# Adttil/crypto12381

Hardware: AMD Instinct MI355X
Metric: G1 scalar-muls/s per MI355X (batch 2^20 per GPU), bit-exact vs CPU (higher is better)
Workload: dtype int64 accumulate over 14x28-bit signed limbs

## Files before the change

crypto12381_amd/csrc/fp.hpp:

```cpp
#pragma once
#include <cstdint>
#include <type_traits>
#include <utility>

#if defined(__HIPCC__)
#include <hip/hip_runtime.h>
#define C12381_HD __host__ __device__ __forceinline__
#define C12381_HDN __host__ __device__ __noinline__ inline
#define C12381_CONST __device__ constexpr
#else
#define C12381_HD inline
#define C12381_HDN inline
#define C12381_CONST constexpr
#endif

#if defined(__HIP_DEVICE_COMPILE__)
#define C12381_LIMB(x) c12381::limb_opaque(x)
namespace c12381 { __device__ __forceinline__ int32_t limb_opaque(int32_t v) { asm("" : "+v"(v)); return v; } }
#else
#define C12381_LIMB(x) (x)
#endif

#include "consts.hpp"

// ... 176 lines not shown
    int64_t acc = 0;
#pragma unroll
    for (int k = 0; k < NL; ++k) {
#pragma unroll
        for (int i = 0; 2 * i < k; ++i) { acc += (int64_t)a2[i] * a.l[k - i]; }
        if ((k & 1) == 0) { acc += (int64_t)a.l[k / 2] * a.l[k / 2]; }
#pragma unroll
        for (int i = 0; i < k; ++i) { acc += (int64_t)m[i] * FP_P[k - i]; }
        m[k] = (int32_t)(((uint32_t)acc * FP_N0) & LMASK);
        acc += (int64_t)m[k] * FP_P[0];
        acc >>= LB;
    }
#pragma unroll
    for (int k = NL; k < 2 * NL - 1; ++k) {
#pragma unroll
        for (int i = k - NL + 1; 2 * i < k; ++i) { acc += (int64_t)a2[i] * a.l[k - i]; }
        if ((k & 1) == 0) { acc += (int64_t)a.l[k / 2] * a.l[k / 2]; }
#pragma unroll
        for (int i = k - NL + 1; i < NL; ++i) { acc += (int64_t)m[i] * FP_P[k - i]; }
        out[k - NL] = C12381_LIMB((int32_t)((uint32_t)acc & LMASK));
        acc >>= LB;
    }
    out[NL - 1] = (int32_t)acc;
#pragma unroll
    for (int i = 0; i < NL; ++i) r.l[i] = out[i];
    C12381_BOUNDS({ double vb = a.vb * a.vb * P_OVER_R + 1.0;
                    double top = vb * TOP_PER_P + 2.0;
                    set_bounds(r, top > 268435456.0 ? top : 268435456.0, vb, "fp_sqr"); })
}

C12381_HD void fp_sqr2(fp& r, const fp& a) {
    C12381_BOUNDS({ fp d;
                    for (int i = 0; i < NL; ++i) d.l[i] = 2 * a.l[i];
                    d.lb = 2 * a.lb; d.vb = 2 * a.vb;
                    check_mul_operands(a, d, "fp_sqr2"); })
    C12381_COUNT(27, 1);
    int32_t m[NL];
    int32_t out[NL];
    int32_t a2[NL];
#pragma unroll
    for (int i = 0; i < NL; ++i) a2[i] = 2 * a.l[i];
    int64_t acc = 0;
#pragma unroll
    for (int k = 0; k < NL; ++k) {
#pragma unroll
        for (int i = 0; 2 * i < k; ++i) { acc += (int64_t)a2[i] * a2[k - i]; }
        if ((k & 1) == 0) { acc += (int64_t)a2[k / 2] * a.l[k / 2]; }
#pragma unroll
        for (int i = 0; i < k; ++i) { acc += (int64_t)m[i] * FP_P[k - i]; }
        m[k] = (int32_t)(((uint32_t)acc * FP_N0) & LMASK);
        acc += (int64_t)m[k] * FP_P[0];
        acc >>= LB;
    }
#pragma unroll
    for (int k = NL; k < 2 * NL - 1; ++k) {
#pragma unroll
        for (int i = k - NL + 1; 2 * i < k; ++i) { acc += (int64_t)a2[i] * a2[k - i]; }
        if ((k & 1) == 0) { acc += (int64_t)a2[k / 2] * a.l[k / 2]; }
#pragma unroll
        for (int i = k - NL + 1; i < NL; ++i) { acc += (int64_t)m[i] * FP_P[k - i]; }
        out[k - NL] = C12381_LIMB((int32_t)((uint32_t)acc & LMASK));
        acc >>= LB;
    }
    out[NL - 1] = (int32_t)acc;
#pragma unroll
    for (int i = 0; i < NL; ++i) r.l[i] = out[i];
    C12381_BOUNDS({ double vb = 2 * a.vb * a.vb * P_OVER_R + 1.0;
                    double top = vb * TOP_PER_P + 2.0;
                    set_bounds(r, top > 268435456.0 ? top : 268435456.0, vb, "fp_sqr2"); })
}

C12381_HD void fp_col_acc(int64_t& acc, const fp& a, const fp& b, int k) {
    C12381_COUNT(1, 0);
#pragma unroll
    for (int i = 0; i < NL; ++i) {
        const int j = k - i;
        if (j >= 0 && j < NL) { acc += (int64_t)a.l[i] * b.l[j]; }
    }
}
C12381_HD void fp_col_sqr_acc(int64_t& acc, const fp& a, const fp& a2, const fp& ad, int k) {
    C12381_COUNT(1, 0);
#pragma unroll
    for (int i = 0; i < NL; ++i) {
        const int j = k - i;
        if (j > i && j < NL) { acc += (int64_t)a2.l[i] * a.l[j]; }
    }
    if ((k & 1) == 0 && k / 2 < NL) { acc += (int64_t)ad.l[k / 2] * a.l[k / 2]; }
}
C12381_HD void fp_raw_neg(fp& r, const fp& a) {
#pragma unroll
    for (int i = 0; i < NL; ++i) r.l[i] = -a.l[i];
    C12381_BOUNDS(r.lb = a.lb; r.vb = a.vb;)
}
C12381_HD void fp_raw_dbl(fp& r, const fp& a) {
#pragma unroll
    for (int i = 0; i < NL; ++i) r.l[i] = 2 * a.l[i];
    C12381_BOUNDS(r.lb = 2 * a.lb; r.vb = 2 * a.vb;)
}
C12381_HD void fp_raw_neg_dbl(fp& r, const fp& a) {
#pragma unroll
    for (int i = 0; i < NL; ++i) r.l[i] = -2 * a.l[i];
    C12381_BOUNDS(r.lb = 2 * a.lb; r.vb = 2 * a.vb;)
}
template <class ColFn>
C12381_HD void fp_reduce_cols(fp& r, ColFn col) {
    C12381_COUNT(0, 1);
    int32_t m[NL];
    int32_t out[NL];
    int64_t acc = 0;
#pragma unroll
    for (int k = 0; k < NL; ++k) {
        col(k, acc);
#pragma unroll
        for (int i = 0; i < k; ++i) { acc += (int64_t)m[i] * FP_P[k - i]; }
        m[k] = (int32_t)(((uint32_t)acc * FP_N0) & LMASK);
        acc += (int64_t)m[k] * FP_P[0];
        acc >>= LB;
    }
#pragma unroll
    for (int k = NL; k < 2 * NL - 1; ++k) {
        col(k, acc);
#pragma unroll
        for (int i = k - NL + 1; i < NL; ++i) { acc += (int64_t)m[i] * FP_P[k - i]; }
        out[k - NL] = C12381_LIMB((int32_t)((uint32_t)acc & LMASK));
        acc >>= LB;
    }
    out[NL - 1] = (int32_t)acc;
#pragma unroll
    for (int i = 0; i < NL; ++i) r.l[i] = out[i];
}
template <int... Ks, class Fn>
C12381_HD void fp_static_for(std::integer_sequence<int, Ks...>, Fn&& fn) { (fn(std::integral_constant<int, Ks>{}), ...); }
template <class ColFn>
C12381_HD void fp_reduce_cols_static(fp& r, ColFn col) {
    C12381_COUNT(0, 1);
    int32_t m[NL];
    int32_t out[NL];
    int64_t acc = 0;
    fp_static_for(std::make_integer_sequence<int, NL>{}, [&](auto kc) {
        constexpr int k = decltype(kc)::value;
        col(k, acc);
#pragma unroll
        for (int i = 0; i < k; ++i) { acc += (int64_t)m[i] * FP_P[k - i]; }
        m[k] = (int32_t)(((uint32_t)acc * FP_N0) & LMASK);
        acc += (int64_t)m[k] * FP_P[0];
        acc >>= LB;
    });
    fp_static_for(std::make_integer_sequence<int, NL - 1>{}, [&](auto kc) {
        constexpr int k = NL + decltype(kc)::value;
        col(k, acc);
#pragma unroll
        for (int i = k - NL + 1; i < NL; ++i) { acc += (int64_t)m[i] * FP_P[k - i]; }
        out[k - NL] = C12381_LIMB((int32_t)((uint32_t)acc & LMASK));
        acc >>= LB;
    });
    out[NL - 1] = (int32_t)acc;
#pragma unroll
    for (int i = 0; i < NL; ++i) r.l[i] = out[i];
}
C12381_HD void fp_inj(int64_t& acc, const fp& c, int i, int32_t k) { acc += (int64_t)c.l[i] * k; }
C12381_HD void fp_inj_p(int64_t& acc, int i, int32_t k) { acc += (int64_t)FP_P[i] * k; }
C12381_HD int32_t fp_quot_top(int32_t top) { return (int32_t)(((int64_t)top * 1321315992 + ((int64_t)1 << 46)) >> 47); }
#if defined(__HIP_DEVICE_COMPILE__)
C12381_HD int32_t fp_opaque_const(int32_t v) { asm("" : "+s"(v)); return v; }
#else
C12381_HD int32_t fp_opaque_const(int32_t v) { return v; }
#endif
template <class ColFn, class InjFn>
C12381_HD void fp_reduce_cols_inj(fp& r, ColFn col, InjFn inj) {
    C12381_COUNT(0, 1);
    int32_t m[NL];
    int32_t out[NL];
    int64_t acc = 0;
#pragma unroll
    for (int k = 0; k < NL; ++k) {
        col(k, acc);
#pragma unroll
        for (int i = 0; i < k; ++i) { acc += (int64_t)m[i] * FP_P[k - i]; }
        m[k] = (int32_t)(((uint32_t)acc * FP_N0) & LMASK);
        acc += (int64_t)m[k] * FP_P[0];
        acc >>= LB;
    }
#pragma unroll
    for (int k = NL; k < 2 * NL - 1; ++k) {
        col(k, acc);
        inj(k - NL, acc);
#pragma unroll
        for (int i = k - NL + 1; i < NL; ++i) { acc += (int64_t)m[i] * FP_P[k - i]; }
        out[k - NL] = C12381_LIMB((int32_t)((uint32_t)acc & LMASK));
        acc >>= LB;
    }
    inj(NL - 1, acc);
    out[NL - 1] = (int32_t)acc;
#pragma unroll
    for (int i = 0; i < NL; ++i) r.l[i] = out[i];
}
template <class InjFn>
C12381_HD void fp_mul_inj(fp& r, const fp& a, const fp& b, InjFn inj, double inj_vb, double inj_lb) {
    C12381_COUNT(27, 0);
    fp t;
    fp_reduce_cols_inj(t, [&](int k, int64_t& acc) {
#pragma unroll
        for (int i = 0; i < NL; ++i) { const int j = k - i; if (j >= 0 && j < NL) { acc += (int64_t)a.l[i] * b.l[j]; } }
    }, inj);
    (void)inj_vb; (void)inj_lb;
    C12381_BOUNDS({ check_actual(a, "fp_mul_inj"); check_actual(b, "fp_mul_inj"); set_inj_bounds(t, a.lb * b.lb, a.vb * b.vb, inj_vb, inj_lb, "fp_mul_inj"); })
    r = t;
}
template <class InjFn>
C12381_HD void fp_sqr_inj(fp& r, const fp& a, InjFn inj, double inj_vb, double inj_lb) {
    C12381_COUNT(27, 0);
    fp t, a2;
    fp_raw_dbl(a2, a);
    fp_reduce_cols_inj(t, [&](int k, int64_t& acc) {
#pragma unroll
        for (int i = 0; i < NL; ++i) { const int j = k - i; if (j > i && j < NL) { acc += (int64_t)a2.l[i] * a.l[j]; } }
        if ((k & 1) == 0 && k / 2 < NL) { acc += (int64_t)a.l[k / 2] * a.l[k / 2]; }
    }, inj);
    (void)inj_vb; (void)inj_lb;
    C12381_BOUNDS({ check_actual(a, "fp_sqr_inj"); set_inj_bounds(t, a.lb * a.lb, a.vb * a.vb, inj_vb, inj_lb, "fp_sqr_inj"); })
    r = t;
}
C12381_HD void fp_norm1_dbl(fp& r, const fp& a) {
    int32_t c[NL];
#pragma unroll
    for (int i = 0; i < NL - 1; ++i) c[i] = a.l[i] >> (LB - 1);
    const int32_t t13 = 2 * a.l[NL - 1] + c[NL - 2];
#pragma unroll
    for (int i = NL - 2; i >= 1; --i) r.l[i] = C12381_LIMB((int32_t)(((uint32_t)a.l[i] << 1) & LMASK)) + c[i - 1];
    r.l[0] = C12381_LIMB((int32_t)(((uint32_t)a.l[0] << 1) & LMASK));
    r.l[NL - 1] = t13;
    C12381_BOUNDS({ double top = 2 * a.vb * TOP_PER_P + 6.0 + std::floor(2 * a.lb / 268435456.0);
                    double lb = 268435456.0 + std::floor(2 * a.lb / 268435456.0) + 1.0;
                    set_bounds(r, lb > top ? lb : top, 2 * a.vb, "fp_norm1_dbl"); })
}

C12381_HD void fp_lincomb3p(fp& r, const fp& a, int32_t k0, const fp& b, int32_t k1, const fp& c, int32_t k2, int32_t kp, double vb) {
    int64_t t = 0;
    int32_t out[NL];
#pragma unroll
    for (int i = 0; i < NL - 1; ++i) {
        t += (int64_t)a.l[i] * k0; t += (int64_t)b.l[i] * k1; t += (int64_t)c.l[i] * k2; t += (int64_t)FP_P[i] * kp;
        out[i] = C12381_LIMB((int32_t)((uint32_t)t & LMASK));
        t >>= LB;
    }
    t += (int64_t)a.l[NL - 1] * k0; t += (int64_t)b.l[NL - 1] * k1; t += (int64_t)c.l[NL - 1] * k2; t += (int64_t)FP_P[NL - 1] * kp;
    out[NL - 1] = (int32_t)t;
#pragma unroll
    for (int i = 0; i < NL; ++i) r.l[i] = out[i];
    (void)vb;
    C12381_BOUNDS({ double top = vb * TOP_PER_P + 2.0;
                    set_bounds(r, top > 268435456.0 ? top : 268435456.0, vb, "fp_lincomb3p"); check_actual_vb(r, "fp_lincomb3p value"); })
}

template <bool SUB>
C12381_HD void fp_mul2(fp& r, const fp& a, const fp& b, const fp& c, const fp& d);

#ifdef C12381_CHECK_BOUNDS
inline void set_lazy_bounds(fp& r, double sum_lblb, double sum_vbvb, const char* where) {
    double col = 14.0 * sum_lblb + 14.0 * 72057594037927936.0 + 1099511627776.0;
    if (col >= 9223372036854775808.0) bounds_fail(where, sum_lblb, sum_vbvb);
    if (sum_vbvb > 1.0e6) bounds_fail("lazy form value bound", sum_vbvb, 0);
    double vb = sum_vbvb * P_OVER_R + 1.0;
    double top = vb * TOP_PER_P + 2.0;
    set_bounds(r, top > 268435456.0 ? top : 268435456.0, vb, where);
}
inline void set_inj_bounds(fp& r, double sum_lblb, double sum_vbvb, double inj_abs, double inj_lb, const char* where) {
    double col = 14.0 * sum_lblb + 14.0 * 72057594037927936.0 + 1099511627776.0 + inj_lb;
    if (col >= 9223372036854775808.0) bounds_fail(where, sum_lblb, inj_lb);
    if (sum_vbvb > 1.0e6) bounds_fail("injected form value bound", sum_vbvb, 0);
    double vb = sum_vbvb * P_OVER_R + 1.0 + inj_abs;
    double top = vb * TOP_PER_P + 2.0;
    set_bounds(r, top > 268435456.0 ? top : 268435456.0, vb, where);
    check_actual_vb(r, where);
}
inline double fp_actual_vb(const fp& a) {
    long double v = 0, w = 1;
    for (int i = 0; i < NL; ++i) { v += (long double)a.l[i] * w; w *= 268435456.0L; }
    long double pp = 0; w = 1;
    for (int i = 0; i < NL; ++i) { pp += (long double)FP_P[i] * w; w *= 268435456.0L; }
    return (double)fabsl(v / pp);
}
inline void check_actual_vb(const fp& a, const char* where) { const double v = fp_actual_vb(a); if (v > a.vb * 1.0000001 + 1e-9) bounds_fail(where, v, a.vb); }
#endif

template <bool SUB>
C12381_HD void fp_mul2(fp& r, const fp& a, const fp& b, const fp& c, const fp& d) {
    fp t, cs;
    if (SUB) fp_raw_neg(cs, c); else cs = c;
    fp_reduce_cols(t, [&](int k, int64_t& acc) { fp_col_acc(acc, a, b, k); fp_col_acc(acc, cs, d, k); });
    C12381_BOUNDS({ check_actual(a, "fp_mul2"); check_actual(b, "fp_mul2"); check_actual(c, "fp_mul2"); check_actual(d, "fp_mul2");
                    set_lazy_bounds(t, a.lb * b.lb + c.lb * d.lb, a.vb * b.vb + c.vb * d.vb, "fp_mul2"); })
    r = t;
}
C12381_HD void fp_mul_msqr2(fp& r, const fp& a, const fp& b, const fp& c) {
    fp t, c2, c4;
    fp_raw_neg_dbl(c2, c);
    fp_raw_dbl(c4, c2);
    fp_reduce_cols(t, [&](int k, int64_t& acc) { fp_col_acc(acc, a, b, k); fp_col_sqr_acc(acc, c, c4, c2, k); });
    C12381_BOUNDS({ check_actual(a, "fp_mul_msqr2"); check_actual(b, "fp_mul_msqr2"); check_actual(c, "fp_mul_msqr2");
                    set_lazy_bounds(t, a.lb * b.lb + 2 * c.lb * c.lb, a.vb * b.vb + 2 * c.vb * c.vb, "fp_mul_msqr2"); })
    r = t;
}

C12381_HD void fp_from_mont_canonical(fp& r, const fp& a) {
    fp one;
    fp_zero(one);
    one.l[0] = 1;
    C12381_BOUNDS(one.lb = 1; one.vb = 1e-100;)
    fp t;
    fp_mul(t, a, one);
    bool eqp = true;
#pragma unroll
    for (int i = 0; i < NL; ++i) eqp = eqp && (t.l[i] == FP_P[i]);
#pragma unroll
    for (int i = 0; i < NL; ++i) r.l[i] = eqp ? 0 : t.l[i];
    C12381_BOUNDS(r.lb = 268435456.0; r.vb = 1.0;)
}
C12381_HD bool fp_is_zero(const fp& a) {
    fp t;
    fp_from_mont_canonical(t, a);
    int32_t o = 0;
#pragma unroll
    for (int i = 0; i < NL; ++i) o |= t.l[i];
    return o == 0;
}
C12381_HD bool fp_equal(const fp& a, const fp& b) {
    fp d;
    fp_sub(d, a, b);
    return fp_is_zero(d);
}

C12381_HD void fp_from_words_be(fp& r, const uint32_t (&w)[12]) {
    fp t;
#pragma unroll
    for (int i = 0; i < NL; ++i) {
        const int bit = i * LB;
        const int wi = bit / 32, sh = bit % 32;
        uint64_t lo = w[11 - wi];
        if (wi + 1 < 12) lo |= (uint64_t)w[11 - (wi + 1)] << 32;
        t.l[i] = C12381_LIMB((int32_t)((uint32_t)(lo >> sh) & LMASK));
    }
    C12381_BOUNDS(t.lb = 268435456.0; t.vb = 10.0;)
    fp r2;
    fp_set_const(r2, FP_R2);
    fp_mul(r, t, r2);
}
C12381_HD void fp_to_words_be(uint32_t (&w)[12], const fp& a) {
    fp t;
    fp_from_mont_canonical(t, a);
#pragma unroll
    for (int j = 0; j < 12; ++j) {
        const int bit = j * 32;
        const int li = bit / LB, sh = bit % LB;
        uint64_t v = (uint64_t)(uint32_t)t.l[li] >> sh;
        if (li + 1 < NL) v |= (uint64_t)(uint32_t)t.l[li + 1] << (LB - sh);
        if (li + 2 < NL && 2 * LB - sh < 32) v |= (uint64_t)(uint32_t)t.l[li + 2] << (2 * LB - sh);
        w[11 - j] = (uint32_t)v;
    }
}
C12381_HD int fp_sign(const fp& a) {
    fp t;
    fp_from_mont_canonical(t, a);
    return t.l[0] & 1;
}

C12381_HDN void fp_pow_fixed(fp& r, const fp& a, const uint32_t (&e)[12]) {
    fp tab[16];
    fp_one(tab[0]);
    {
        fp n;
        fp_norm1(n, a);
        tab[1] = n;
    }
#pragma unroll 1
    for (int i = 2; i < 16; ++i) fp_mul(tab[i], tab[i - 1], tab[1]);
    fp acc;
    fp_one(acc);
#pragma unroll 1
    for (int wi = 95; wi >= 0; --wi) {
        fp_sqr(acc, acc); fp_sqr(acc, acc); fp_sqr(acc, acc); fp_sqr(acc, acc);
        const uint32_t d = (e[wi / 8] >> (4 * (wi % 8))) & 15u;
        fp_mul(acc, acc, tab[d]);
    }
    r = acc;
}
C12381_HD void fp_inv_fermat(fp& r, const fp& a) { fp_pow_fixed(r, a, EXP_P_MINUS_2); }

constexpr int SG_N = 13;
struct sg30 { int32_t v[SG_N]; };
C12381_HD int32_t sg_divsteps_30(int32_t zeta, uint32_t f0, uint32_t g0, int32_t (&t)[4]) {
    uint32_t u = 1, v = 0, q = 0, r = 1, f = f0, g = g0;
#pragma unroll 1
    for (int i = 0; i < 30; ++i) {
        uint32_t c1 = (uint32_t)(zeta >> 31);
        const uint32_t c2 = (uint32_t)0 - (g & 1u);
        const uint32_t x = (f ^ c1) - c1, y = (u ^ c1) - c1, z = (v ^ c1) - c1;
        g += x & c2; q += y & c2; r += z & c2;
        c1 &= c2;
        zeta = (int32_t)((uint32_t)zeta ^ c1) - 1;
        f += g & c1; u += q & c1; v += r & c1;
        g >>= 1; u <<= 1; v <<= 1;
    }
    t[0] = (int32_t)u; t[1] = (int32_t)v; t[2] = (int32_t)q; t[3] = (int32_t)r;
    return zeta;
}
C12381_HD void sg_update_de(sg30& d, sg30& e, const int32_t (&t)[4]) {
    constexpr int32_t M30 = (int32_t)0x3fffffff;
    const int32_t u = t[0], v = t[1], q = t[2], r = t[3];
    const int32_t sd = d.v[SG_N - 1] >> 31, se = e.v[SG_N - 1] >> 31;
    int32_t md = (u & sd) + (v & se), me = (q & sd) + (r & se);
    int32_t di = d.v[0], ei = e.v[0];
    int64_t cd = (int64_t)u * di + (int64_t)v * ei;
    int64_t ce = (int64_t)q * di + (int64_t)r * ei;
    md -= (int32_t)((SG_PINV30 * (uint32_t)cd + (uint32_t)md) & (uint32_t)M30);
    me -= (int32_t)((SG_PINV30 * (uint32_t)ce + (uint32_t)me) & (uint32_t)M30);
    cd += (int64_t)SG_P30[0] * md;
    ce += (int64_t)SG_P30[0] * me;
    cd >>= 30; ce >>= 30;
#pragma unroll
    for (int i = 1; i < SG_N; ++i) {
        di = d.v[i]; ei = e.v[i];
        cd += (int64_t)u * di + (int64_t)v * ei;
        ce += (int64_t)q * di + (int64_t)r * ei;
        cd += (int64_t)SG_P30[i] * md;
        ce += (int64_t)SG_P30[i] * me;
        d.v[i - 1] = (int32_t)cd & M30; cd >>= 30;
        e.v[i - 1] = (int32_t)ce & M30; ce >>= 30;
    }
    d.v[SG_N - 1] = (int32_t)cd; e.v[SG_N - 1] = (int32_t)ce;
}
C12381_HD void sg_update_fg(sg30& f, sg30& g, const int32_t (&t)[4]) {
    constexpr int32_t M30 = (int32_t)0x3fffffff;
    const int32_t u = t[0], v = t[1], q = t[2], r = t[3];
    int32_t fi = f.v[0], gi = g.v[0];
    int64_t cf = (int64_t)u * fi + (int64_t)v * gi;
    int64_t cg = (int64_t)q * fi + (int64_t)r * gi;
    cf >>= 30; cg >>= 30;
#pragma unroll
    for (int i = 1; i < SG_N; ++i) {
        fi = f.v[i]; gi = g.v[i];
        cf += (int64_t)u * fi + (int64_t)v * gi;
        cg += (int64_t)q * fi + (int64_t)r * gi;
        f.v[i - 1] = (int32_t)cf & M30; cf >>= 30;
        g.v[i - 1] = (int32_t)cg & M30; cg >>= 30;
    }
    f.v[SG_N - 1] = (int32_t)cf; g.v[SG_N - 1] = (int32_t)cg;
}
C12381_HD void sg_normalize(sg30& r, int32_t sign) {
    constexpr int32_t M30 = (int32_t)0x3fffffff;
    int32_t w[SG_N];
#pragma unroll
    for (int i = 0; i < SG_N; ++i) w[i] = r.v[i];
    int32_t cond_add = w[SG_N - 1] >> 31;
#pragma unroll
    for (int i = 0; i < SG_N; ++i) w[i] += SG_P30[i] & cond_add;
    const int32_t cond_negate = sign >> 31;
#pragma unroll
    for (int i = 0; i < SG_N; ++i) w[i] = (w[i] ^ cond_negate) - cond_negate;
#pragma unroll
    for (int i = 0; i < SG_N - 1; ++i) { w[i + 1] += w[i] >> 30; w[i] &= M30; }
    cond_add = w[SG_N - 1] >> 31;
#pragma unroll
    for (int i = 0; i < SG_N; ++i) w[i] += SG_P30[i] & cond_add;
#pragma unroll
    for (int i = 0; i < SG_N - 1; ++i) { w[i + 1] += w[i] >> 30; w[i] &= M30; }
#pragma unroll
    for (int i = 0; i < SG_N; ++i) r.v[i] = w[i];
}
C12381_HDN void fp_inv_divsteps(fp& r, const fp& a) {
    fp c;
    fp_from_mont_canonical(c, a);
    sg30 d, e, f, g;
#pragma unroll
    for (int j = 0; j < SG_N; ++j) {
        const int bit = 30 * j, li = bit / LB, sh = bit % LB;
        uint64_t v = (uint64_t)(uint32_t)c.l[li] >> sh;
        if (li + 1 < NL) v |= (uint64_t)(uint32_t)c.l[li + 1] << (LB - sh);
        if (li + 2 < NL && 2 * LB - sh < 30) v |= (uint64_t)(uint32_t)c.l[li + 2] << (2 * LB - sh);
        g.v[j] = (int32_t)((uint32_t)v & 0x3fffffffu);
        f.v[j] = SG_P30[j];
        d.v[j] = 0; e.v[j] = 0;
    }
    e.v[0] = 1;
    int32_t zeta = -1;
#pragma unroll 1
    for (int it = 0; it < 30; ++it) {
        int32_t t[4];
        zeta = sg_divsteps_30(zeta, (uint32_t)f.v[0], (uint32_t)g.v[0], t);
        sg_update_de(d, e, t);
        sg_update_fg(f, g, t);
    }
    sg_normalize(d, f.v[SG_N - 1]);
    fp x;
#pragma unroll
    for (int i = 0; i < NL; ++i) {
        const int bit = LB * i, li = bit / 30, sh = bit % 30;
        uint64_t v = (uint64_t)(uint32_t)d.v[li] >> sh;
        if (li + 1 < SG_N) v |= (uint64_t)(uint32_t)d.v[li + 1] << (30 - sh);
        x.l[i] = C12381_LIMB((int32_t)((uint32_t)v & LMASK));
    }
    C12381_BOUNDS(x.lb = 268435456.0; x.vb = 1.0;)
    fp r2;
    fp_set_const(r2, FP_R2);
    fp_mul(r, x, r2);
}
C12381_HD void fp_inv(fp& r, const fp& a) {
    fp_inv_divsteps(r, a);
}
C12381_HD void fp_sqrt_candidate(fp& r, const fp& a) { fp_pow_fixed(r, a, EXP_P_PLUS_1_DIV_4); }
C12381_HD bool fp_sqrt_progen(fp& c, fp& cinv, const fp& a) {
    fp h, an, chi, one, d;
    fp_norm1(an, a);
    fp_pow_fixed(h, an, EXP_P_MINUS_3_DIV_4);
    fp_mul(c, h, an);
    fp_mul(chi, c, h);
    fp_one(one);
    fp_sub(d, chi, one);
    const bool qr = fp_is_zero(d);
    fp nh;
    fp_neg(nh, h);
    fp_select(cinv, qr, h, nh);
    return qr;
}

}
```

crypto12381_amd/csrc/g1.hpp:

```cpp
#pragma once
#include "fp.hpp"

namespace c12381 {

struct g1p { fp x, y, z; };

C12381_HD void g1_set_inf(g1p& p) { fp_zero(p.x); fp_one(p.y); fp_zero(p.z); }
C12381_HD bool g1_is_inf(const g1p& p) { return fp_is_zero(p.z); }
C12381_HD void g1_norm1(g1p& r, const g1p& p) { fp_norm1(r.x, p.x); fp_norm1(r.y, p.y); fp_norm1(r.z, p.z); }
C12381_HD void g1_norm1(g1p& p) { g1_norm1(p, p); }
C12381_HD void g1_select(g1p& r, bool c, const g1p& a, const g1p& b) { fp_select(r.x, c, a.x, b.x); fp_select(r.y, c, a.y, b.y); fp_select(r.z, c, a.z, b.z); }
C12381_HD void g1_set_invalid(g1p& p) { fp_one(p.x); fp_zero(p.y); fp_zero(p.z); }
C12381_HD bool g1_is_invalid(const g1p& p) { return fp_is_zero(p.z) && !fp_is_zero(p.x); }

C12381_HD void g1_dbl(g1p& p) {
    fp t0, t1, t2, z8, u, y3, x3, z3;
    const int32_t cm3 = fp_opaque_const(-3);
    fp_mul(t1, p.y, p.z);
    fp_sqr(t2, p.z);
    fp_mul_small(t2, t2, 12);
    fp_sqr_inj(u, p.y, [&](int i, int64_t& acc) { fp_inj(acc, t2, i, cm3); }, C12381_BV(3 * t2.vb), C12381_BV(3 * t2.lb));
    fp_dbl(t0, t2); fp_add(t0, t0, t2); fp_add(t0, t0, u);
    fp_mul_small(z8, t0, 8);
    fp_add(y3, t0, t2);
// ... 378 lines not shown
    g1_dbl(t);
    g1_norm1(t);
    tab_store_g1(lane_tab + G1_ENT_DWORDS, t);
#pragma unroll 1
    for (int j = 3; j <= G1_TAB; ++j) {
        if ((j & 1) == 0) {
            tab_load_g1(t, lane_tab + (j / 2 - 1) * G1_ENT_DWORDS);
            g1_dbl(t);
        } else {
            g1_add(t, base);
        }
        g1_norm1(t);
        tab_store_g1(lane_tab + (j - 1) * G1_ENT_DWORDS, t);
    }

    g1_digit_point(acc, lane_tab, glv_digit(kb0, G1_WINDOWS - 1), false);
    g1_norm1(acc);
    g1_add_digit(acc, lane_tab, glv_digit(kb1, G1_WINDOWS - 1), true);
#pragma unroll 1
    for (int w = G1_WINDOWS - 2; w >= 0; --w) {
        const int d0 = glv_digit(kb0, w), d1 = glv_digit(kb1, w);
        g1p q0, q1, e;
        tab_load_g1(q0, g1_digit_entry(lane_tab, d0));
        g1_sched_fence();
#pragma unroll 1
        for (int j = 0; j < G1_WIN; ++j) g1_dbl(acc);
        tab_load_g1(q1, g1_digit_entry(lane_tab, d1));
        g1_sched_fence();
        g1_digit_fix(e, q0, d0, false);
        g1_add(acc, e);
        g1_digit_fix(e, q1, d1, true);
        g1_add(acc, e);
    }
}

C12381_HD void tab_load_xy(fp& x, fp& y, const int32_t* ent) {
    int32_t w[G1_ENT_DWORDS];
    tab_load_q4<0, 7>(w, ent);
    rec_field(x, w, 0, 4.0); rec_field(y, w, NL, 4.0);
}
C12381_HD void tab_load_ybx(fp& y, fp& bx, const int32_t* ent) {
    int32_t w[G1_ENT_DWORDS];
    tab_load_q4<3, 8>(w, ent);
    rec_field(y, w, NL, 4.0); rec_field(bx, w, 2 * NL, 4.0);
}
C12381_HD void tab_fetch_xy(fp& x, fp& y, const int32_t* lane_tab, int d) { tab_load_xy(x, y, g1_digit_entry(lane_tab, d)); g1_sched_fence(); }
C12381_HD void tab_fetch_ybx(fp& y, fp& bx, const int32_t* lane_tab, int d) { tab_load_ybx(y, bx, g1_digit_entry(lane_tab, d)); g1_sched_fence(); }
C12381_HD void tab_store_zt(int32_t* lane_tab, const fp& zt) {
#pragma unroll
    for (int j = 0; j < NL / 2; ++j) { d2 t; t.v[0] = zt.l[2 * j]; t.v[1] = zt.l[2 * j + 1]; *reinterpret_cast<d2*>(lane_tab + j * G1_ENT_DWORDS + 42) = t; }
}
C12381_HD void tab_load_zt(fp& zt, const int32_t* lane_tab) {
#pragma unroll
    for (int j = 0; j < NL / 2; ++j) { const d2 t = *reinterpret_cast<const d2*>(lane_tab + j * G1_ENT_DWORDS + 42); zt.l[2 * j] = t.v[0]; zt.l[2 * j + 1] = t.v[1]; }
    C12381_BOUNDS(zt.lb = G1_REC_LB; zt.vb = 4.0; check_actual(zt, "tab_load_zt");)
}

template <class OnH>
C12381_HD void g1_coz_forward(int32_t* lane_tab, const fp& px, const fp& py, const fp& beta, const OnH& on_h) {
    fp x1, y1, xj, yj, xn, yn, h, hn, bx;
    g1j_dblu(xj, yj, x1, y1, px, py);
#pragma unroll 1
    for (int j = 2; j < G1_TAB; ++j) {
        g1j_zaddu(xn, yn, x1, y1, h, xj, yj);
        fp_norm1(hn, h);
        tab_store_rec(lane_tab + (j - 1) * G1_ENT_DWORDS, xj, yj, hn, 32.0);
        on_h(j, hn);
        xj = xn; yj = yn;
    }
    fp_mul(bx, xj, beta);
    tab_store_rec(lane_tab + (G1_TAB - 1) * G1_ENT_DWORDS, xj, yj, bx, 4.0);
    fp_mul(bx, x1, beta);
    tab_store_rec(lane_tab, x1, y1, bx, 4.0);
}
template <bool KEEP_PADS>
C12381_HD void g1_coz_backward(int32_t* ent, fp& mu, bool first, const fp& beta) {
    fp m2, m3, x, y, h, bx;
    tab_load_rec(x, y, h, ent, 32.0);
    if (first) mu = h; else fp_mul(mu, mu, h);
    fp_sqr(m2, mu);
    fp_mul(m3, m2, mu);
    fp_mul(x, x, m2);
    fp_mul(y, y, m3);
    fp_mul(bx, x, beta);
    tab_store_rec<KEEP_PADS>(ent, x, y, bx, 4.0);
}
C12381_HD void g1j_dbl_window(g1j& a) { g1j_dbl(a); g1j_dbl(a); g1j_dbl(a); g1j_dbl(a); g1j_dbl(a); }

C12381_HD void g1j_add_signed(g1j& acc, bool& acc_inf, const fp& x, const fp& y, bool neg, bool keep);
C12381_HD void g1j_add_digit(g1j& acc, bool& acc_inf, const fp& x, const fp& y, int d, bool endo) {
    g1j_add_signed(acc, acc_inf, x, y, (d < 0) != endo, d == 0);
}
C12381_HD void g1j_add_signed(g1j& acc, bool& acc_inf, const fp& x, const fp& y, bool neg, bool keep) {
    fp ny, ys, one;
    fp_neg(ny, y);
    fp_select(ys, neg, ny, y);
    g1j r;
    g1j_madd(r, acc, x, ys);
    fp_one(one);
    fp_select(r.x, acc_inf, x, r.x); fp_select(r.y, acc_inf, ys, r.y); fp_select(r.z, acc_inf, one, r.z);
    fp_select(acc.x, keep, acc.x, r.x); fp_select(acc.y, keep, acc.y, r.y); fp_select(acc.z, keep, acc.z, r.z);
    acc_inf = acc_inf && keep;
}
C12381_HD bool g1_coz_finish(g1p& acc, const g1j& a, const fp& zc, bool inf) {
    fp z, z2;
    fp_mul(z, a.z, zc);
    const bool exc = !inf && fp_is_zero(z);
    fp_sqr(z2, z);
    fp_mul(acc.x, a.x, z);
    acc.y = a.y;
    fp_mul(acc.z, z2, z);
    g1p o;
    g1_set_inf(o);
    g1_select(acc, inf, o, acc);
    return exc;
}

C12381_HD bool g1_scalar_mul(g1p& acc, const fp& px, const fp& py, bool p_is_inf, const uint32_t (&kin)[8], int32_t* lane_tab) {
    uint32_t kb0[5], kb1[5];
    glv_scalar_digits(kb0, kb1, kin);

    fp beta;
    fp_set_const(beta, FP_BETA_A);
    g1_coz_forward(lane_tab, px, py, beta, [](int, const fp&) {});
    {
        fp mu, zt, y2;
#pragma unroll 1
        for (int j = G1_TAB - 1; j >= 2; --j) g1_coz_backward<false>(lane_tab + (j - 1) * G1_ENT_DWORDS, mu, j == G1_TAB - 1, beta);
        fp_raw_dbl(y2, py);
        fp_mul(zt, mu, y2);
        tab_store_zt(lane_tab, zt);
    }

    g1j a;
    bool acc_inf;
    {
        const int d0 = glv_digit(kb0, G1_WINDOWS - 1);
        fp x, y, ny;
        tab_load_xy(x, y, g1_digit_entry(lane_tab, d0));
        fp_neg(ny, y);
        a.x = x;
        fp_select(a.y, d0 < 0, ny, y);
        fp_one(a.z);
        acc_inf = d0 == 0;
        const int d1 = glv_digit(kb1, G1_WINDOWS - 1);
        tab_load_ybx(y, x, g1_digit_entry(lane_tab, d1));
        g1j_add_digit(a, acc_inf, x, y, d1, true);
    }
#pragma unroll 1
    for (int w = G1_WINDOWS - 2; w >= 0; --w) {
        const int d0 = glv_digit(kb0, w), d1 = glv_digit(kb1, w);
        fp x0, y0, x1, y1;
        tab_fetch_xy(x0, y0, lane_tab, d0);
        g1j_dbl_window(a);
        tab_fetch_ybx(y1, x1, lane_tab, d1);
        g1j_add_digit(a, acc_inf, x0, y0, d0, false);
        g1j_add_digit(a, acc_inf, x1, y1, d1, true);
    }

    fp zt;
    tab_load_zt(zt, lane_tab);
    const bool exc = g1_coz_finish(acc, a, zt, acc_inf || p_is_inf);
    if (exc) g1_scalar_mul_complete(acc, px, py, p_is_inf, kin, lane_tab);
    return exc;
}
constexpr int G1E_TAB = 11;
constexpr int G1E_DIGITS = 44;
constexpr uint32_t G1E_NONE = 15;
constexpr int EIS_REPS[G1E_TAB][2] = {{1, 0}, {2, -1}, {2, -2}, {2, -3}, {1, -3}, {0, -3}, {1, -4}, {2, -4}, {3, -5}, {3, -4}, {4, -4}};
struct eis_z { int a, b; };
constexpr eis_z eis_mul_unit(eis_z z, int u) {
    for (int i = 0; i < u; ++i) z = eis_z{-z.b, z.a + z.b};
    return z;
}
constexpr int eis_chain_unit(int i) {
    for (int u = 0; u < 6; ++u) {
        const eis_z w = eis_mul_unit(eis_z{1, 0}, u);
        if (EIS_REPS[i + 1][0] - EIS_REPS[i][0] == w.a && EIS_REPS[i + 1][1] - EIS_REPS[i][1] == w.b) return u;
    }
    return -1;
}
constexpr uint32_t eis_chain_deltas() {
    uint32_t v = 0;
    int prev = 0;
    for (int i = 0; i + 1 < G1E_TAB; ++i) {
        const int u = eis_chain_unit(i);
        v |= (uint32_t)((u - prev + 6) % 6) << (3 * i);
        prev = u;
    }
    return v;
}
constexpr bool eis_chain_ok() {
    for (int i = 0; i + 1 < G1E_TAB; ++i) if (eis_chain_unit(i) < 0) return false;
    return eis_chain_unit(G1E_TAB - 2) == 0;
}
static_assert(eis_chain_ok(), "the representatives are not a chain of unit steps that ends on +P");
constexpr uint32_t EIS_CHAIN_DELTAS = eis_chain_deltas();
struct eis_classes { uint16_t v[64]; };
constexpr eis_classes eis_make_classes() {
    eis_classes t{};
    for (int c = 0; c < 64; ++c) t.v[c] = 0xffff;
    t.v[0] = (uint16_t)G1E_NONE;
    for (int e = 0; e < G1E_TAB; ++e)
        for (int u = 0; u < 6; ++u) {
            const eis_z d = eis_mul_unit(eis_z{EIS_REPS[e][0], EIS_REPS[e][1]}, u);
            const int c = (d.a & 7) + 8 * (d.b & 7);
            if (t.v[c] == 0xffff && d.a >= -5 && d.a <= 5 && d.b >= -5 && d.b <= 5)
                t.v[c] = (uint16_t)(e | (u << 4) | ((d.a < 0 ? 1 : 0) << 7) | ((d.b < 0 ? 1 : 0) << 8));
        }
    return t;
}
constexpr bool eis_classes_ok(const eis_classes& t) {
    for (int c = 0; c < 64; ++c) if (t.v[c] == 0xffff) return false;
    return true;
}
C12381_CONST eis_classes EIS_CLASSES = eis_make_classes();
static_assert(eis_classes_ok(eis_make_classes()), "a class mod 8 without a representative");
constexpr uint32_t eis_exact_code(int a, int b) {
    const uint32_t c = eis_make_classes().v[(a & 7) + 8 * (b & 7)] & 127u;
    if ((c & 15u) >= (uint32_t)G1E_TAB) return 0xffu;
    const eis_z d = eis_mul_unit(eis_z{EIS_REPS[c & 15u][0], EIS_REPS[c & 15u][1]}, (int)(c >> 4));
    return d.a == a && d.b == b ? c : 0xffu;
}
constexpr uint32_t EIS_TOP_ONE = eis_exact_code(1, 0), EIS_TOP_PSI = eis_exact_code(0, 1);
constexpr uint32_t EIS_LOW_ONE = eis_exact_code(-5, 2), EIS_LOW_PSI = eis_exact_code(3, -5);
constexpr uint32_t EIS_SEED_ONE = eis_exact_code(2, 2), EIS_SEED_PSI = eis_exact_code(2, 3);
static_assert(EIS_TOP_ONE == 0u && EIS_TOP_PSI == 16u, "1 and psi are not entry 0 under the units 0 and 1");
static_assert(EIS_LOW_ONE != 0xffu && EIS_LOW_PSI != 0xffu, "the digits under a non-empty top position are not (-5, 2) and (3, -5)");
static_assert(EIS_SEED_ONE != 0xffu && EIS_SEED_PSI != 0xffu, "the table does not hold (2, 2) and (2, 3) themselves");

C12381_HD void eis_next(uint32_t (&c)[4], uint32_t t) {
    uint64_t s = t;
#pragma unroll
    for (int i = 0; i < 4; ++i) { s += (c[i] >> 3) | (i < 3 ? c[i + 1] << 29 : 0u); c[i] = (uint32_t)s; s >>= 32; }
}
C12381_HD void eis_recode(uint32_t (&kd)[10], const uint32_t (&k0)[4], const uint32_t (&k1)[4]) {
    uint32_t a[4], b[4];
#pragma unroll
    for (int i = 0; i < 4; ++i) { a[i] = k0[i]; b[i] = k1[i]; }
#pragma unroll
    for (int i = 0; i < 10; ++i) kd[i] = 0;
#pragma unroll
    for (int n = 0; n < G1E_DIGITS; ++n) {
        const uint32_t e = EIS_CLASSES.v[(a[0] & 7u) | ((b[0] & 7u) << 3)];
        const int pos = 7 * (G1E_DIGITS - 1 - n), word = pos >> 5, sh = pos & 31;
        kd[word] |= (e & 127u) << sh;
        if (sh > 25) kd[word + 1] |= (e & 127u) >> (32 - sh);
        eis_next(a, (e >> 7) & 1u);
        eis_next(b, (e >> 8) & 1u);
    }
}
C12381_HD void eis_scalar_digits(uint32_t (&kd)[10], const uint32_t (&kin)[8]) {
    uint32_t k[8], k0[4], k1[4];
#pragma unroll
    for (int i = 0; i < 8; ++i) k[i] = kin[i];
    scalar_mod_r(k);
    scalar_glv_split(k0, k1, k);
    eis_recode(kd, k0, k1);
}
C12381_HD uint32_t eis_pop_digit(uint32_t (&kd)[10]) {
    const uint32_t d = kd[0] & 127u;
#pragma unroll
    for (int i = 0; i < 10; ++i) kd[i] = (kd[i] >> 7) | (i < 9 ? kd[i + 1] << 25 : 0u);
    return d;
}

constexpr int G1E_FIELD = 16;
constexpr int G1E_ENT_DWORDS = 4 * G1E_FIELD;
static_assert(G1E_TAB * G1E_ENT_DWORDS == G1_TAB_DWORDS, "the Eisenstein table fills the lane's record of the 16-entry table");
C12381_HD void eis_store_field(int32_t* ent, int f, const fp& a, double vb_cap) {
    (void)vb_cap;
    C12381_BOUNDS(if (a.vb > vb_cap) bounds_fail("eis_store_field value bound", a.vb, vb_cap);
                  if (a.lb > G1_REC_LB) bounds_fail("eis_store_field limb bound", a.lb, G1_REC_LB);)
    int32_t w[G1E_FIELD];
#pragma unroll
    for (int i = 0; i < NL; ++i) w[i] = a.l[i];
    w[14] = 0; w[15] = 0;
    rec_store_q4<0, G1E_FIELD / 4>(reinterpret_cast<q4*>(ent + f * G1E_FIELD), w);
}
C12381_HD void eis_load_field(fp& a, const int32_t* ent, int f, double vb_cap) {
    int32_t w[G1E_FIELD];
    rec_load_q4<0, G1E_FIELD / 4>(w, reinterpret_cast<const q4*>(ent + f * G1E_FIELD));
#pragma unroll
    for (int i = 0; i < NL; ++i) a.l[i] = w[i];
    (void)vb_cap;
    C12381_BOUNDS(a.lb = G1_REC_LB; a.vb = vb_cap; check_actual(a, "eis_load_field");)
}
C12381_HD void eis_store_zt(int32_t* lane_tab, const fp& zt) {
#pragma unroll
    for (int j = 0; j < NL / 2; ++j) { d2 t; t.v[0] = zt.l[2 * j]; t.v[1] = zt.l[2 * j + 1]; *reinterpret_cast<d2*>(lane_tab + j * G1E_ENT_DWORDS + NL) = t; }
}
C12381_HD void eis_load_zt(fp& zt, const int32_t* lane_tab) {
#pragma unroll
    for (int j = 0; j < NL / 2; ++j) { const d2 t = *reinterpret_cast<const d2*>(lane_tab + j * G1E_ENT_DWORDS + NL); zt.l[2 * j] = t.v[0]; zt.l[2 * j + 1] = t.v[1]; }
    C12381_BOUNDS(zt.lb = G1_REC_LB; zt.vb = 4.0; check_actual(zt, "eis_load_zt");)
}
C12381_HD void eis_fetch(fp& x, fp& y, const int32_t* lane_tab, uint32_t code) {
    const uint32_t e = code & 15u, u = code >> 4;
    const int32_t* ent = lane_tab + (e >= (uint32_t)G1E_TAB ? 0u : e) * G1E_ENT_DWORDS;
    eis_load_field(y, ent, 0, 4.0);
    eis_load_field(x, ent, 1 + (int)(u >= 3u ? u - 3u : u), 4.0);
    g1_sched_fence();
}
C12381_HD void g1j_add_eis(g1j& acc, bool& acc_inf, const fp& x, const fp& y, uint32_t code) {
    g1j_add_signed(acc, acc_inf, x, y, ((code >> 4) & 1u) != 0u, (code & 15u) == G1E_NONE);
}

C12381_HD void g1e_forward(int32_t* lane_tab, const fp& px, const fp& py, const fp& beta, const fp& beta2) {
    fp x1 = px, y1 = py, xj = px, yj = py, xn, yn, h, hn, bx;
#pragma unroll 1
    for (int i = 0; i + 1 < G1E_TAB; ++i) {
        const uint32_t dl = (EIS_CHAIN_DELTAS >> (3 * i)) & 7u, m = dl >= 3u ? dl - 3u : dl;
        if (m != 0u) {
            fp bm;
            fp_select(bm, m == 2u, beta2, beta);
            fp_mul(x1, x1, bm);
        }
        if (dl & 1u) fp_neg(y1, y1);
        g1j_zaddu(xn, yn, x1, y1, h, xj, yj);
        fp_norm1(hn, h);
        int32_t* ent = lane_tab + i * G1E_ENT_DWORDS;
        eis_store_field(ent, 0, yj, 32.0); eis_store_field(ent, 1, xj, 32.0); eis_store_field(ent, 2, hn, 32.0);
        xj = xn; yj = yn;
    }
    int32_t* last = lane_tab + (G1E_TAB - 1) * G1E_ENT_DWORDS;
    eis_store_field(last, 0, yj, 4.0); eis_store_field(last, 1, xj, 4.0);
    fp_mul(bx, xj, beta); eis_store_field(last, 2, bx, 4.0);
    fp_mul(bx, xj, beta2); eis_store_field(last, 3, bx, 4.0);
    eis_store_field(lane_tab, 0, y1, 4.0); eis_store_field(lane_tab, 1, x1, 4.0);
    fp_mul(bx, x1, beta2); eis_store_field(lane_tab, 3, bx, 4.0);
}
C12381_HD void g1e_backward(int32_t* ent, fp& mu, bool first, const fp& beta, const fp& beta2) {
    fp m2, m3, x, y, h, bx;
    eis_load_field(y, ent, 0, 32.0); eis_load_field(x, ent, 1, 32.0); eis_load_field(h, ent, 2, 32.0);
    if (first) mu = h; else fp_mul(mu, mu, h);
    fp_sqr(m2, mu);
    fp_mul(m3, m2, mu);
    fp_mul(x, x, m2);
    fp_mul(y, y, m3);
    eis_store_field(ent, 0, y, 4.0); eis_store_field(ent, 1, x, 4.0);
    fp_mul(bx, x, beta); eis_store_field(ent, 2, bx, 4.0);
    fp_mul(bx, x, beta2); eis_store_field(ent, 3, bx, 4.0);
}
C12381_HD void g1e_add_affine(g1j& r, const fp& x1, const fp& y1, const fp& x2, const fp& y2) {
    fp h, s, hh, hhh, v, x3, y3, vx;
    const int32_t cm1 = fp_opaque_const(-1), cm2 = fp_opaque_const(-2);
    fp_sub(h, x2, x1);
    fp_sub(s, y2, y1);
    fp_sqr(hh, h);
    fp_mul(hhh, h, hh);
    fp_mul(v, x1, hh);
    fp_sqr_inj(x3, s, [&](int i, int64_t& acc) { fp_inj(acc, hhh, i, cm1); fp_inj(acc, v, i, cm2); },
               C12381_BV(hhh.vb + 2 * v.vb), C12381_BV(hhh.lb + 2 * v.lb));
    fp_sub(vx, v, x3);
    fp_mul2<true>(y3, s, vx, y1, hhh);
    r.x = x3; r.y = y3;
    fp_norm1(r.z, h);
}

C12381_HD bool g1_scalar_mul_eis(g1p& acc, const fp& px, const fp& py, bool p_is_inf, const uint32_t (&kin)[8], int32_t* lane_tab) {
    uint32_t kd[10];
    eis_scalar_digits(kd, kin);

    fp beta, beta2;
    fp_set_const(beta, FP_BETA_A);
    fp_set_const(beta2, FP_BETA_B);
    g1e_forward(lane_tab, px, py, beta, beta2);
    {
        fp mu, zt, h0, x, bx;
#pragma unroll 1
        for (int i = G1E_TAB - 2; i >= 1; --i) g1e_backward(lane_tab + i * G1E_ENT_DWORDS, mu, i == G1E_TAB - 2, beta, beta2);
        eis_load_field(h0, lane_tab, 2, 32.0);
        eis_load_field(x, lane_tab, 1, 4.0);
        fp_mul(zt, mu, h0);
        fp_mul(bx, x, beta);
        eis_store_field(lane_tab, 2, bx, 4.0);
        eis_store_zt(lane_tab, zt);
    }

    g1j a;
    bool acc_inf;
    {
        const uint32_t top = eis_pop_digit(kd), low = eis_pop_digit(kd);
        const bool two = (top & 15u) != G1E_NONE;
        C12381_BOUNDS(if (two && !(top == EIS_TOP_ONE && low == EIS_LOW_ONE) && !(top == EIS_TOP_PSI && low == EIS_LOW_PSI))
                          bounds_fail("the top two digits are no pair the seed knows", top, low);)
        const uint32_t code = two ? (top == EIS_TOP_ONE ? EIS_SEED_ONE : EIS_SEED_PSI) : low;
        fp x, y, ny, ys, x0, y0, one;
        eis_load_field(y0, lane_tab, 0, 4.0); eis_load_field(x0, lane_tab, 1, 4.0);
        eis_fetch(x, y, lane_tab, code);
        fp_neg(ny, y);
        fp_select(ys, ((code >> 4) & 1u) != 0u, ny, y);
        g1e_add_affine(a, x, ys, x0, y0);
        fp_one(one);
        fp_select(a.x, two, a.x, x); fp_select(a.y, two, a.y, ys); fp_select(a.z, two, a.z, one);
        acc_inf = (code & 15u) == G1E_NONE;
    }
#pragma unroll 1
    for (int w = G1E_DIGITS - 3; w >= 0; --w) {
        const uint32_t code = eis_pop_digit(kd);
        fp x, y;
        eis_fetch(x, y, lane_tab, code);
        g1j_dbl(a); g1j_dbl(a); g1j_dbl(a);
        g1j_add_eis(a, acc_inf, x, y, code);
    }

    fp zt;
    eis_load_zt(zt, lane_tab);
    const bool exc = g1_coz_finish(acc, a, zt, acc_inf || p_is_inf);
    if (exc) g1_scalar_mul_complete(acc, px, py, p_is_inf, kin, lane_tab);
    return exc;
}
C12381_HD void tab_store_kb(int32_t* lane_tab, const uint32_t (&kb0)[5], const uint32_t (&kb1)[5]) {
#pragma unroll
    for (int j = 0; j < 5; ++j) { d2 t; t.v[0] = (int32_t)kb0[j]; t.v[1] = (int32_t)kb1[j]; *reinterpret_cast<d2*>(lane_tab + (NL / 2 + j) * G1_ENT_DWORDS + 42) = t; }
}
C12381_HD void tab_load_kb(uint32_t (&kb0)[5], uint32_t (&kb1)[5], const int32_t* lane_tab) {
#pragma unroll
    for (int j = 0; j < 5; ++j) { const d2 t = *reinterpret_cast<const d2*>(lane_tab + (NL / 2 + j) * G1_ENT_DWORDS + 42); kb0[j] = (uint32_t)t.v[0]; kb1[j] = (uint32_t)t.v[1]; }
}

template <int K, class In>
C12381_HD bool g1_scalar_mul_sum(g1p& acc, const In& in, int32_t* lane_tab) {
    static_assert(K >= 1 && K <= 4, "terms per lane");
    fp beta;
    fp_set_const(beta, FP_BETA_A);
#pragma unroll 1
    for (int t = 0; t < K; ++t) {
        int32_t* tab = lane_tab + t * G1_TAB_DWORDS;
        fp px, py;
        bool p_is_inf;
        uint32_t k[8], kb0[5], kb1[5];
        in(t, px, py, p_is_inf, k);
        glv_scalar_digits(kb0, kb1, k, p_is_inf);
        fp zrun, zt, y2, one;
        g1_coz_forward(tab, px, py, beta, [&](int j, const fp& hn) { if (j == 2) zrun = hn; else fp_mul(zrun, zrun, hn); });
        fp_raw_dbl(y2, py);
        fp_mul(zt, zrun, y2);
        fp_one(one);
        fp_select(zt, p_is_inf, one, zt);
        tab_store_zt(tab, zt);
        tab_store_kb(tab, kb0, kb1);
    }
#pragma unroll 1
    for (int t = 0; t < K; ++t) {
        int32_t* tab = lane_tab + t * G1_TAB_DWORDS;
        fp mu;
        if (K > 1) {
            fp m2, m3, x, y, h, bx;
            bool first = true;
#pragma unroll 1
            for (int l = 0; l < K; ++l) {
                if (l == t) continue;
                tab_load_zt(h, lane_tab + l * G1_TAB_DWORDS);
                if (first) mu = h; else fp_mul(mu, mu, h);
                first = false;
            }
            fp_sqr(m2, mu);
            fp_mul(m3, m2, mu);
#pragma unroll 1
            for (int e = 0; e < 2; ++e) {
                int32_t* ent = tab + (e == 0 ? 0 : G1_TAB - 1) * G1_ENT_DWORDS;
                tab_load_rec(x, y, bx, ent, 4.0);
                fp_mul(x, x, m2);
                fp_mul(y, y, m3);
                fp_mul(bx, bx, m2);
                tab_store_rec<true>(ent, x, y, bx, 4.0);
            }
        }
#pragma unroll 1
        for (int j = G1_TAB - 1; j >= 2; --j) g1_coz_backward<true>(tab + (j - 1) * G1_ENT_DWORDS, mu, K == 1 && j == G1_TAB - 1, beta);
    }

    uint32_t kb[2 * K][5];
#pragma unroll
    for (int t = 0; t < K; ++t) tab_load_kb(kb[2 * t], kb[2 * t + 1], lane_tab + t * G1_TAB_DWORDS);
    g1j a;
    fp_one(a.x); a.y = a.x; a.z = a.x;
    bool acc_inf = true;
#pragma unroll 1
    for (int w = G1_WINDOWS - 1; w >= 0; --w) {
        fp x0, y0, x1, y1;
        int d0 = glv_digit(kb[0], w);
        tab_fetch_xy(x0, y0, lane_tab, d0);
        if (w < G1_WINDOWS - 1) g1j_dbl_window(a);
        const int32_t* tab = lane_tab;
#pragma unroll 1
        for (int t = 0; t < K; ++t) {
            const int d1 = glv_digit(kb[1], w);
            tab_fetch_ybx(y1, x1, tab, d1);
            g1j_add_digit(a, acc_inf, x0, y0, d0, false);
            if (K > 1) {
#pragma unroll
                for (int i = 0; i < 5; ++i) {
                    const uint32_t r0 = kb[0][i], r1 = kb[1][i];
#pragma unroll
                    for (int j = 0; j + 2 < 2 * K; ++j) kb[j][i] = kb[j + 2][i];
                    kb[2 * K - 2][i] = r0; kb[2 * K - 1][i] = r1;
                }
                tab += G1_TAB_DWORDS;
                if (t + 1 < K) {
                    d0 = glv_digit(kb[0], w);
                    tab_fetch_xy(x0, y0, tab, d0);
                }
            }
            g1j_add_digit(a, acc_inf, x1, y1, d1, true);
        }
    }

    fp zc, z;
    tab_load_zt(zc, lane_tab);
#pragma unroll 1
    for (int t = 1; t < K; ++t) {
        tab_load_zt(z, lane_tab + t * G1_TAB_DWORDS);
        fp_mul(zc, zc, z);
    }
    const bool exc = g1_coz_finish(acc, a, zc, acc_inf);
    if (exc) {
#pragma unroll 1
        for (int t = 0; t < K; ++t) {
            fp px, py;
            bool p_is_inf;
            uint32_t k[8];
            in(t, px, py, p_is_inf, k);
            g1p term, n;
            g1_scalar_mul_complete(term, px, py, p_is_inf, k, lane_tab);
            g1_norm1(n, term);
            if (t == 0) { acc = n; continue; }
            g1_add(acc, n);
            g1_norm1(acc);
        }
    }
    return exc;
}
C12381_HD bool scalar_below_x2(const uint32_t (&kin)[8]) {
    uint32_t k[8];
#pragma unroll
    for (int i = 0; i < 8; ++i) k[i] = kin[i];
    scalar_mod_r(k);
    uint64_t bw = 0;
#pragma unroll
    for (int i = 0; i < 4; ++i) { uint64_t t = (uint64_t)k[i] - GLV_X2[i] - bw; bw = (t >> 32) & 1; }
    return (k[4] | k[5] | k[6] | k[7]) == 0u && bw == 1;
}

C12381_HD void g1_to_affine(fp& ax, fp& ay, const g1p& p, const fp& zinv) {
    fp_mul(ax, p.x, zinv);
    fp_mul(ay, p.y, zinv);
}

C12381_HD bool g1_set_x(fp& y, const fp& x, int s) {
    fp x2, x3, four, rhs, c, cinv, ny;
    fp_sqr(x2, x); fp_mul(x3, x2, x);
    fp_set_const(four, FP_FOUR);
    fp_add(rhs, x3, four);
    const bool qr = fp_sqrt_progen(c, cinv, rhs);
    fp_neg(ny, c);
    fp_select(y, fp_sign(c) != s, ny, c);
    return qr;
}

}
```

Measured before the change: 53.21 million.

## Use custom mixed-add formula and replace beta2 multiplies with negated sums

```diff
diff --git a/crypto12381_amd/csrc/fp.hpp b/crypto12381_amd/csrc/fp.hpp
--- a/crypto12381_amd/csrc/fp.hpp
+++ b/crypto12381_amd/csrc/fp.hpp
@@ -502,6 +502,15 @@
                     set_lazy_bounds(t, a.lb * b.lb + 2 * c.lb * c.lb, a.vb * b.vb + 2 * c.vb * c.vb, "fp_mul_msqr2"); })
     r = t;
 }
+C12381_HD void fp_sqr_mmul(fp& r, const fp& a, const fp& b, const fp& c) {
+    fp t, a2, bn;
+    fp_raw_dbl(a2, a);
+    fp_raw_neg(bn, b);
+    fp_reduce_cols(t, [&](int k, int64_t& acc) { fp_col_sqr_acc(acc, a, a2, a, k); fp_col_acc(acc, bn, c, k); });
+    C12381_BOUNDS({ check_actual(a, "fp_sqr_mmul"); check_actual(b, "fp_sqr_mmul"); check_actual(c, "fp_sqr_mmul");
+                    set_lazy_bounds(t, a.lb * a.lb + b.lb * c.lb, a.vb * a.vb + b.vb * c.vb, "fp_sqr_mmul"); })
+    r = t;
+}
 
 C12381_HD void fp_from_mont_canonical(fp& r, const fp& a) {
     fp one;
diff --git a/crypto12381_amd/csrc/g1.hpp b/crypto12381_amd/csrc/g1.hpp
--- a/crypto12381_amd/csrc/g1.hpp
+++ b/crypto12381_amd/csrc/g1.hpp
@@ -704,10 +704,45 @@
     eis_load_field(x, ent, 1 + (int)(u >= 3u ? u - 3u : u), 4.0);
     g1_sched_fence();
 }
+C12381_HD void g1j_madd_eis(g1j& r, const g1j& p, const fp& x2, const fp& y2) {
+    fp zz, zzz, u2, s2, h, s, hh, nhh, ux, tn, x3, y3, z3;
+    fp_sqr(zz, p.z);
+    fp_mul(u2, x2, zz);
+    fp_mul(zzz, p.z, zz);
+    fp_mul(s2, y2, zzz);
+    fp_sub(h, u2, p.x);
+    fp_sub(s, s2, p.y);
+    fp_mul(z3, p.z, h);
+    fp_sqr(hh, h);
+    fp_add(ux, u2, p.x);
+    fp_sqr_mmul(x3, s, hh, ux);
+    fp_mul2<true>(tn, p.y, h, s, p.x);
+    fp_raw_neg(nhh, hh);
+    fp_mul2<true>(y3, nhh, tn, s, x3);
+    r.x = x3; r.y = y3; r.z = z3;
+}
+C12381_HD void g1j_add_signed_eis(g1j& acc, bool& acc_inf, const fp& x, const fp& y, bool neg, bool keep) {
+    fp ny, ys, one;
+    fp_neg(ny, y);
+    fp_select(ys, neg, ny, y);
+    g1j r;
+    g1j_madd_eis(r, acc, x, ys);
+    fp_one(one);
+    fp_select(r.x, acc_inf, x, r.x); fp_select(r.y, acc_inf, ys, r.y); fp_select(r.z, acc_inf, one, r.z);
+    fp_select(acc.x, keep, acc.x, r.x); fp_select(acc.y, keep, acc.y, r.y); fp_select(acc.z, keep, acc.z, r.z);
+    acc_inf = acc_inf && keep;
+}
 C12381_HD void g1j_add_eis(g1j& acc, bool& acc_inf, const fp& x, const fp& y, uint32_t code) {
-    g1j_add_signed(acc, acc_inf, x, y, ((code >> 4) & 1u) != 0u, (code & 15u) == G1E_NONE);
-}
-
+    g1j_add_signed_eis(acc, acc_inf, x, y, ((code >> 4) & 1u) != 0u, (code & 15u) == G1E_NONE);
+}
+
+constexpr double G1E_X0_VB = 2.0;
+C12381_HD void eis_beta2_sum(fp& r, const fp& x, const fp& bx) {
+    fp t;
+    fp_add(t, x, bx);
+    fp_neg(t, t);
+    fp_norm1(r, t);
+}
 C12381_HD void g1e_forward(int32_t* lane_tab, const fp& px, const fp& py, const fp& beta, const fp& beta2) {
     fp x1 = px, y1 = py, xj = px, yj = py, xn, yn, h, hn, bx;
 #pragma unroll 1
@@ -729,10 +764,9 @@
     eis_store_field(last, 0, yj, 4.0); eis_store_field(last, 1, xj, 4.0);
     fp_mul(bx, xj, beta); eis_store_field(last, 2, bx, 4.0);
     fp_mul(bx, xj, beta2); eis_store_field(last, 3, bx, 4.0);
-    eis_store_field(lane_tab, 0, y1, 4.0); eis_store_field(lane_tab, 1, x1, 4.0);
-    fp_mul(bx, x1, beta2); eis_store_field(lane_tab, 3, bx, 4.0);
-}
-C12381_HD void g1e_backward(int32_t* ent, fp& mu, bool first, const fp& beta, const fp& beta2) {
+    eis_store_field(lane_tab, 0, y1, 4.0); eis_store_field(lane_tab, 1, x1, G1E_X0_VB);
+}
+C12381_HD void g1e_backward(int32_t* ent, fp& mu, bool first, const fp& beta) {
     fp m2, m3, x, y, h, bx;
     eis_load_field(y, ent, 0, 32.0); eis_load_field(x, ent, 1, 32.0); eis_load_field(h, ent, 2, 32.0);
     if (first) mu = h; else fp_mul(mu, mu, h);
@@ -742,7 +776,24 @@
     fp_mul(y, y, m3);
     eis_store_field(ent, 0, y, 4.0); eis_store_field(ent, 1, x, 4.0);
     fp_mul(bx, x, beta); eis_store_field(ent, 2, bx, 4.0);
-    fp_mul(bx, x, beta2); eis_store_field(ent, 3, bx, 4.0);
+    eis_beta2_sum(bx, x, bx); eis_store_field(ent, 3, bx, 4.0);
+}
+C12381_HD void g1e_table(int32_t* lane_tab, const fp& px, const fp& py) {
+    fp beta, beta2;
+    fp_set_const(beta, FP_BETA_A);
+    fp_set_const(beta2, FP_BETA_B);
+    g1e_forward(lane_tab, px, py, beta, beta2);
+    fp mu, zt, h0, x, bx;
+#pragma unroll 1
+    for (int i = G1E_TAB - 2; i >= 1; --i) g1e_backward(lane_tab + i * G1E_ENT_DWORDS, mu, i == G1E_TAB - 2, beta);
+    eis_load_field(h0, lane_tab, 2, 32.0);
+    eis_load_field(x, lane_tab, 1, G1E_X0_VB);
+    fp_mul(zt, mu, h0);
+    fp_mul(bx, x, beta);
+    eis_store_field(lane_tab, 2, bx, 4.0);
+    eis_beta2_sum(bx, x, bx);
+    eis_store_field(lane_tab, 3, bx, 4.0);
+    eis_store_zt(lane_tab, zt);
 }
 C12381_HD void g1e_add_affine(g1j& r, const fp& x1, const fp& y1, const fp& x2, const fp& y2) {
     fp h, s, hh, hhh, v, x3, y3, vx;
@@ -764,21 +815,7 @@
     uint32_t kd[10];
     eis_scalar_digits(kd, kin);
 
-    fp beta, beta2;
-    fp_set_const(beta, FP_BETA_A);
-    fp_set_const(beta2, FP_BETA_B);
-    g1e_forward(lane_tab, px, py, beta, beta2);
-    {
-        fp mu, zt, h0, x, bx;
-#pragma unroll 1
-        for (int i = G1E_TAB - 2; i >= 1; --i) g1e_backward(lane_tab + i * G1E_ENT_DWORDS, mu, i == G1E_TAB - 2, beta, beta2);
-        eis_load_field(h0, lane_tab, 2, 32.0);
-        eis_load_field(x, lane_tab, 1, 4.0);
-        fp_mul(zt, mu, h0);
-        fp_mul(bx, x, beta);
-        eis_store_field(lane_tab, 2, bx, 4.0);
-        eis_store_zt(lane_tab, zt);
-    }
+    g1e_table(lane_tab, px, py);
 
     g1j a;
     bool acc_inf;
```

Result: no change. 53.72 million, median of 6 (+1.0%).
